# ishika28/Beyond-Binary-Fake-User-Detection-A-Credibility-Aware-Graph-based-Recommender-System

Measured on AMD Instinct MI355X. Metric: SpMM edges/sec + BPR steps/sec, |E|=50M d=64, 1/2/4/8 MI355X; %HBM roofline, higher is better.
Workload: dtype f32

## Files before the change

beyond-binary-fake-user-detection-a-credibility-aware-graph-based-recommender-system_amd/_lib.py:

```python
from __future__ import annotations

import ctypes
import os
import re
from pathlib import Path

import torch

PKG_DIR = Path(__file__).resolve().parent
LIB_PATH = Path(os.environ.get("BBGR_LIB", PKG_DIR / "lib" / "libbbgr.so"))
HEADER_PATH = PKG_DIR.parent / "include" / "bbgr.h"

BBGR_OK = 0
STATUS = {0: "BBGR_OK", -1: "BBGR_ERR_INVALID", -2: "BBGR_ERR_UNSUPPORTED",
          -3: "BBGR_ERR_HIP", -4: "BBGR_ERR_WORKSPACE"}

OP_GS, OP_METHOD_A, OP_J, OP_SYM = 0, 1, 2, 3
NEG_CAP = 65536

c_int32 = ctypes.c_int32
c_int64 = ctypes.c_int64
c_float = ctypes.c_float
c_double = ctypes.c_double
c_void_p = ctypes.c_void_p
# ... 211 lines not shown
        ("side", c_void_p), ("side_bytes", c_int64),
        ("n_records", c_int64), ("user_bytes", c_int64), ("item_bytes", c_int64),
        ("text_bytes", c_int64),
        ("out_rating", c_void_p), ("out_helpful", c_void_p), ("out_verified", c_void_p),
        ("out_timestamp", c_void_p), ("out_ts_valid", c_void_p),
        ("user_data", c_void_p), ("user_off", c_void_p),
        ("item_data", c_void_p), ("item_off", c_void_p),
        ("text_data", c_void_p), ("text_off", c_void_p),
    ]


class Pcg64State(ctypes.Structure):
    _fields_ = [
        ("state_hi", c_uint64), ("state_lo", c_uint64),
        ("inc_hi", c_uint64), ("inc_lo", c_uint64),
        ("has_uint32", c_int32), ("uinteger", ctypes.c_uint32),
    ]


class BatchArgs(ctypes.Structure):
    _fields_ = [
        ("batch", c_int64), ("users", c_void_p), ("pos", c_void_p), ("neg", c_void_p),
        ("n_users", c_int64), ("n_items", c_int64),
        ("user_indptr", c_void_p), ("user_indices", c_void_p),
        ("mask_u", c_void_p), ("mask_i", c_void_p),
        ("list", c_void_p), ("count", c_void_p),
        ("slot_map", c_void_p), ("slot_bits", c_void_p),
        ("g_u", c_void_p), ("g_i", c_void_p), ("g_side", c_void_p),
        ("ld_gu", c_int64), ("ld_gi", c_int64), ("ld_side", c_int64),
        ("d", c_int32),
    ]


class RowsMarkArgs(ctypes.Structure):
    _fields_ = [
        ("n_users_listed", c_int64), ("n_items_listed", c_int64),
        ("users", c_void_p), ("items", c_void_p),
        ("n_users", c_int64), ("n_items", c_int64),
        ("user_rank", c_void_p), ("item_rank", c_void_p),
        ("user_indptr", c_void_p), ("user_indices", c_void_p),
        ("mask_u", c_void_p), ("mask_i", c_void_p), ("frontier", c_void_p),
        ("mask_u_in", c_void_p), ("mask_i_in", c_void_p),
        ("user_list", c_void_p), ("user_count", c_void_p),
        ("frontier_list", c_void_p), ("frontier_count", c_void_p),
    ]


_P = c_void_p
_SIGNATURES = {
    "bbgr_abi_version": ([], c_int32),
    "bbgr_last_error": ([], ctypes.c_char_p),
    "bbgr_device_info": ([ctypes.c_int, _P, ctypes.c_char_p, ctypes.c_int], c_int32),
    "bbgr_sync": ([_P], c_int32),
    "bbgr_profile_marker": ([c_int32, _P], c_int32),
    "bbgr_csr_build": ([c_int64, _P, _P, c_int32, c_int32, _P, _P, _P, _P,
                        ctypes.POINTER(c_size_t), _P], c_int32),
    "bbgr_csr_plan_count": ([ctypes.POINTER(CsrStruct), ctypes.POINTER(c_int32),
                             ctypes.POINTER(c_int32), _P, ctypes.POINTER(c_size_t), _P],
                            c_int32),
    "bbgr_csr_plan_build": ([ctypes.POINTER(CsrStruct), _P, _P, _P,
                             ctypes.POINTER(c_size_t), _P], c_int32),
    "bbgr_operator_scales": ([c_int32, c_int32, c_int32, _P, _P, _P, _P, _P, _P, _P,
                              _P, _P, _P, _P, _P], c_int32),
    "bbgr_gather_scale": ([c_int64, _P, _P, _P, _P], c_int32),
    "bbgr_degree_count": ([c_int64, _P, c_int32, _P, _P], c_int32),
    "bbgr_degree_count_ws": ([c_int64, _P, c_int32, _P, _P, ctypes.POINTER(c_size_t), _P],
                             c_int32),
    "bbgr_degree_order": ([c_int32, _P, _P, _P, _P, ctypes.POINTER(c_size_t), _P], c_int32),
    "bbgr_relabel": ([c_int64, _P, _P, _P, _P], c_int32),
    "bbgr_spmm": ([ctypes.POINTER(CsrStruct), ctypes.POINTER(SpmmArgs), _P], c_int32),
    "bbgr_epilogue": ([c_int32, _P, c_int64, ctypes.POINTER(SpmmArgs), _P], c_int32),
    "bbgr_to_bf16": ([c_int64, c_int32, _P, c_int64, _P, c_int64, _P], c_int32),
    "bbgr_spmm_bf16": ([ctypes.POINTER(CsrStruct), ctypes.POINTER(SpmmArgs),
                        ctypes.POINTER(SpmmBf16Io), _P], c_int32),
    "bbgr_bpr": ([ctypes.POINTER(BprArgs), _P], c_int32),
    "bbgr_bpr_reduce": ([c_int64, _P, c_float, c_float, _P, _P], c_int32),
    "bbgr_adam": ([c_int64, _P, _P, _P, _P, c_float, c_double, c_double, c_float,
                   c_float, c_float, c_float, c_float, _P], c_int32),
    "bbgr_adam_dev": ([c_int64, _P, _P, _P, _P, c_float, c_double, c_double, c_float,
                       c_float, c_float, _P, _P, _P], c_int32),
    "bbgr_step_begin": ([_P, _P], c_int32),
    "bbgr_mark_rows": ([c_int64, _P, ctypes.c_uint8, _P, c_int64, _P], c_int32),
    "bbgr_comm_unique_id": ([_P], c_int32),
    "bbgr_comm_init": ([_P, c_int32, c_int32, _P], c_int32),
    "bbgr_comm_destroy": ([_P], c_int32),
    "bbgr_allreduce_items": ([_P, _P, c_int64, _P], c_int32),
    "bbgr_comm_allreduce": ([_P, _P, c_int64, c_int32, c_int32, _P], c_int32),
    "bbgr_comm_allgather": ([_P, _P, _P, c_int64, c_int32, _P], c_int32),
    "bbgr_ewa_normalize": ([ctypes.POINTER(CsrStruct), _P, _P, _P, _P, c_int64, c_int32, c_int32,
                            c_float, c_float, c_float, _P, _P, _P, _P,
                            ctypes.POINTER(c_size_t), _P], c_int32),
    "bbgr_scatter_add_rows": ([c_int64, _P, _P, c_int64, _P, c_int64, c_int32, c_int64, _P,
                               ctypes.POINTER(c_size_t), _P], c_int32),
    "bbgr_scatter_plan": ([c_int64, _P, c_int64, _P, ctypes.POINTER(c_size_t), _P], c_int32),
    "bbgr_scatter_apply": ([c_int64, c_int64, _P, _P, c_int64, _P, c_int64, _P, c_int64, c_int32,
                            _P], c_int32),
    "bbgr_mark_neighbors": ([c_int64, _P, _P, _P, ctypes.c_uint8, _P, _P], c_int32),
    "bbgr_mark_slots": ([c_int64, _P, _P, _P, _P, c_int32, _P], c_int32),
    "bbgr_batch_begin": ([ctypes.POINTER(BatchArgs), _P], c_int32),
    "bbgr_mask_pack": ([c_int64, _P, _P, _P], c_int32),
    "bbgr_batch_end": ([ctypes.POINTER(BatchArgs), _P], c_int32),
    "bbgr_rows_mark": ([ctypes.POINTER(RowsMarkArgs), _P], c_int32),
    "bbgr_mark_list": ([c_int64, _P, _P, _P, _P, c_int64, _P, _P, _P], c_int32),
    "bbgr_slots_from_perms": ([c_int64, _P, _P, _P, _P, _P], c_int32),
    "bbgr_transpose_slots": ([ctypes.POINTER(CsrStruct), ctypes.POINTER(CsrStruct), _P, _P],
                             c_int32),
    "bbgr_mark_neighbors_of_mask": ([c_int64, _P, _P, _P, _P, ctypes.c_uint8, _P, _P],
                                    c_int32),
    "bbgr_row_support": ([c_int64, c_int32, _P, c_int64, _P, _P, _P, _P, _P], c_int32),
    "bbgr_rows_zero": ([c_int64, _P, _P, c_int64, c_int32, _P], c_int32),
    "bbgr_rows_axpy": ([c_int64, _P, c_float, _P, c_int64, _P, c_int64, c_int32, _P],
                       c_int32),
    "bbgr_pop_cdf": ([c_int32, _P, c_double, _P, _P, ctypes.POINTER(c_size_t), _P],
                     c_int32),
# ... 165 lines not shown
```

beyond-binary-fake-user-detection-a-credibility-aware-graph-based-recommender-system_amd/csrc/common.h:

```cpp
#pragma once

#include <hip/hip_runtime.h>
#include <stdint.h>
#include <stdio.h>
#include <string>
#include <type_traits>

#include "bbgr.h"

namespace bbgr {

void set_error(const char *fmt, ...);

inline int hip_fail(hipError_t e, const char *what) {
  set_error("%s: %s", what, hipGetErrorString(e));
  return BBGR_ERR_HIP;
}

#define BBGR_HIP(call)                                                        \
  do {                                                                        \
    hipError_t e_ = (call);                                                   \
    if (e_ != hipSuccess) return ::bbgr::hip_fail(e_, #call);                 \
  } while (0)

// ... 94 lines not shown
    case 8: return f(std::integral_constant<int, 8>{});
    case 16: return f(std::integral_constant<int, 16>{});
    case 32: return f(std::integral_constant<int, 32>{});
    case 64: return f(std::integral_constant<int, 64>{});
    case 128: return f(std::integral_constant<int, 128>{});
    default: return f(std::integral_constant<int, 256>{});
  }
}

template <typename F> inline auto for_wide_width(int d, F &&f) {
  switch (d) {
    case 64: return f(std::integral_constant<int, 64>{});
    case 128: return f(std::integral_constant<int, 128>{});
    default: return f(std::integral_constant<int, 256>{});
  }
}

typedef float f4v __attribute__((ext_vector_type(4)));
__device__ __forceinline__ float4 ld_nt(const float4 *p) {
  const f4v v = __builtin_nontemporal_load(reinterpret_cast<const f4v *>(p));
  return make_float4(v.x, v.y, v.z, v.w);
}
__device__ __forceinline__ int ld_nt(const int *p) { return __builtin_nontemporal_load(p); }
__device__ __forceinline__ float ld_nt(const float *p) { return __builtin_nontemporal_load(p); }
__device__ __forceinline__ void st_nt(float4 *p, float4 v) {
  f4v w;
  w.x = v.x;
  w.y = v.y;
  w.z = v.z;
  w.w = v.w;
  __builtin_nontemporal_store(w, reinterpret_cast<f4v *>(p));
}

struct AdamConsts {
  float step;
  float w1;
  float b2;
  float w2;
  float eps;
  float wd;
  float bc2s;
};

__host__ __device__ inline AdamConsts adam_consts(float lr, double b1, double b2, float eps,
                                                  float wd, float bc1, float bc2s) {
  return AdamConsts{lr / bc1, (float)(1.0 - b1), (float)b2, (float)(1.0 - b2), eps, wd, bc2s};
}

__device__ __forceinline__ void adam_elem(float &p, float g, float &m, float &v,
                                          const AdamConsts &c) {
#pragma clang fp contract(off)
  if (c.wd != 0.f) g = fmaf(c.wd, p, g);
  m = fmaf(c.w1, g - m, m);
  v = fmaf(c.w2 * g, g, v * c.b2);
  const float denom = sqrtf(v) / c.bc2s + c.eps;
  p = fmaf(-c.step, m / denom, p);
}

__device__ __forceinline__ long clamp_step(const long *state) {
  const long t = state[0], n = state[3];
  return t < 1 ? 1 : (t > n ? n : t);
}

__host__ __device__ __forceinline__ int plan_chunks(long deg, int thr, int chunk) {
  return deg > thr ? (int)((deg + chunk - 1) / chunk) : 0;
}

}
```

beyond-binary-fake-user-detection-a-credibility-aware-graph-based-recommender-system_amd/csrc/train.hip:

```cpp
#include <hipcub/hipcub.hpp>

#include "common.h"

namespace bbgr {

struct BprParams {
  long batch, n_users, n_items;
  const long *users, *pos, *neg;
  const float *uf, *itf, *ue, *ie;
  long lduf, ldif, ldue, ldie;
  const float *pop;
  float reg, lambda_fair, inv_b;
  float *parts;
  const float *dloss;
  float *g_uf, *g_if, *g_ue, *g_ie;
  long ldguf, ldgif, ldgue, ldgie;
  float *contrib;
  long ldc;
  float *scores_out;
  const float *scores;
};

__device__ __forceinline__ float group16_sum(float v) {
  v += __shfl_xor(v, 1, 16);
// ... 214 lines not shown
#pragma unroll
    for (int u = 0; u < ADAM_TILE; ++u) {
      const long k = t0 + u * 256 + threadIdx.x;
      if (k < n4) {
        pp[u] = ld_nt(p + k);
        gg[u] = ld_nt(g + k);
        mm[u] = ld_nt(m + k);
        vv[u] = ld_nt(v + k);
      }
    }
#pragma unroll
    for (int u = 0; u < ADAM_TILE; ++u) {
      const long k = t0 + u * 256 + threadIdx.x;
      if (k < n4) {
        adam_elem(pp[u].x, gs * gg[u].x, mm[u].x, vv[u].x, c);
        adam_elem(pp[u].y, gs * gg[u].y, mm[u].y, vv[u].y, c);
        adam_elem(pp[u].z, gs * gg[u].z, mm[u].z, vv[u].z, c);
        adam_elem(pp[u].w, gs * gg[u].w, mm[u].w, vv[u].w, c);
        st_nt(p + k, pp[u]);
        st_nt(m + k, mm[u]);
        st_nt(v + k, vv[u]);
      }
    }
  }
}

__global__ void adam_tail_kernel(long n, long start, float *p, const float *g, float *m,
                                 float *v, AdamConsts c0, float gs, float lr, const float *bc,
                                 const long *state) {
  const long i = start + (long)blockIdx.x * blockDim.x + threadIdx.x;
  if (i >= n) return;
  const AdamConsts c = device_step_consts(c0, lr, bc, state);
  adam_elem(p[i], gs * g[i], m[i], v[i], c);
}

__global__ void step_begin_kernel(long *state) {
  if (threadIdx.x != 0 || blockIdx.x != 0) return;
  const long t = state[0], next = state[2];
  state[0] = t + 1;
  state[1] = next;
  state[2] = next + 1;
}

__global__ void rows_zero_kernel(long n, const long *idx, float *t, long ld,
                                 int d) {
  const long k = (long)blockIdx.x * (blockDim.x / 16) + (threadIdx.x >> 4);
  if (k >= n || idx[k] < 0) return;
  float *row = t + idx[k] * ld;
  for (int c = threadIdx.x & 15; c < d; c += 16) row[c] = 0.f;
}

__global__ void mark_rows_kernel(long n, const long *idx, unsigned char v,
                                 unsigned char *mask, long n_rows) {
  const long k = (long)blockIdx.x * blockDim.x + threadIdx.x;
  if (k >= n) return;
  const long r = idx[k];
  if (r >= 0 && r < n_rows) mask[r] = v;
}

__global__ void mark_neighbors_kernel(long n, const long *rows, const int *indptr,
                                      const int *indices, unsigned char v,
                                      unsigned char *mask) {
  const long k = (long)blockIdx.x * (blockDim.x / 16) + (threadIdx.x >> 4);
  if (k >= n || rows[k] < 0) return;
  const long r = rows[k];
  for (int e = indptr[r] + (threadIdx.x & 15); e < indptr[r + 1]; e += 16)
// ... 708 lines not shown
                       dim3(256), 0, st, (long)n, start, param, grad, exp_avg,
                       exp_avg_sq, c, grad_scale, lr, bc, state);
    BBGR_LAUNCHED("adam_tail_kernel");
  }
  return BBGR_OK;
}

extern "C" int bbgr_adam(int64_t n, float *param, const float *grad,
                         float *exp_avg, float *exp_avg_sq, float lr, double beta1,
                         double beta2, float eps, float weight_decay, float grad_scale,
                         float bias_correction1, float bias_correction2_sqrt,
                         bbgr_stream_t stream) {
  BBGR_REQUIRE(n >= 0, "bbgr_adam: negative n");
  if (n == 0) return BBGR_OK;
  BBGR_REQUIRE(param && grad && exp_avg && exp_avg_sq, "bbgr_adam: null tensor");
  return adam_launch(n, param, grad, exp_avg, exp_avg_sq, lr, beta1, beta2, eps, weight_decay,
                     grad_scale, bias_correction1, bias_correction2_sqrt, nullptr, nullptr,
                     as_stream(stream));
}

extern "C" int bbgr_adam_dev(int64_t n, float *param, const float *grad, float *exp_avg,
                             float *exp_avg_sq, float lr, double beta1, double beta2,
                             float eps, float weight_decay, float grad_scale,
                             const float *bc_table, const int64_t *state,
                             bbgr_stream_t stream) {
  BBGR_REQUIRE(n >= 0, "bbgr_adam_dev: negative n");
  if (n == 0) return BBGR_OK;
  BBGR_REQUIRE(param && grad && exp_avg && exp_avg_sq && bc_table && state,
               "bbgr_adam_dev: null tensor / table / state");
  return adam_launch(n, param, grad, exp_avg, exp_avg_sq, lr, beta1, beta2, eps, weight_decay,
                     grad_scale, 1.f, 1.f, bc_table, (const long *)state, as_stream(stream));
}

extern "C" int bbgr_step_begin(int64_t *state, bbgr_stream_t stream) {
  BBGR_REQUIRE(state, "bbgr_step_begin: null state");
  hipLaunchKernelGGL(step_begin_kernel, dim3(1), dim3(64), 0, as_stream(stream), (long *)state);
  BBGR_LAUNCHED("step_begin_kernel");
  return BBGR_OK;
}

extern "C" int bbgr_rows_zero(int64_t n, const int64_t *idx, float *table,
                              int64_t ld, int32_t d, bbgr_stream_t stream) {
  BBGR_REQUIRE(n >= 0 && d > 0 && ld >= d, "bbgr_rows_zero: bad sizes");
  if (n == 0) return BBGR_OK;
  BBGR_REQUIRE(idx && table, "bbgr_rows_zero: null arrays");
  hipLaunchKernelGGL(rows_zero_kernel, dim3((unsigned)((n + 15) / 16)), dim3(256), 0,
                     as_stream(stream), (long)n, (const long *)idx, table, (long)ld, d);
  BBGR_LAUNCHED("rows_zero_kernel");
  return BBGR_OK;
}

extern "C" int bbgr_mark_rows(int64_t n, const int64_t *idx, uint8_t value,
                              uint8_t *mask, int64_t n_rows, bbgr_stream_t stream) {
  BBGR_REQUIRE(n >= 0 && n_rows >= 0, "bbgr_mark_rows: negative n / n_rows");
  if (n == 0) return BBGR_OK;
  BBGR_REQUIRE(idx && mask, "bbgr_mark_rows: null arrays");
  hipLaunchKernelGGL(mark_rows_kernel, dim3((unsigned)((n + 255) / 256)), dim3(256), 0,
                     as_stream(stream), (long)n, (const long *)idx, value, mask, (long)n_rows);
  BBGR_LAUNCHED("mark_rows_kernel");
  return BBGR_OK;
}

extern "C" int bbgr_mark_neighbors(int64_t n, const int64_t *rows,
                                   const int32_t *indptr, const int32_t *indices,
                                   uint8_t value, uint8_t *mask, bbgr_stream_t stream) {
  BBGR_REQUIRE(n >= 0, "bbgr_mark_neighbors: negative n");
// ... 377 lines not shown
```

beyond-binary-fake-user-detection-a-credibility-aware-graph-based-recommender-system_amd/trainer.py:

```python
from __future__ import annotations

import ctypes
import os

import numpy as np
import torch

from . import _lib
from ._lib import OP_GS, OP_J, OP_METHOD_A, OP_SYM, call, ld, ptr, stream_handle
from .bpr import bpr_args
from .graph import BipartiteGraph, Csr
from .optim import AdamRows, DeviceStepState, adam_step
from .propagate import ORDER_GS, ORDER_J, ListLength, OperatorPair, backward, forward
from .sampler import PopMixSampler, nonempty_rows, shuffle
from .scatter import RowScatter

VARIANTS = {
    "v2_pop": (OP_GS, ORDER_GS, 0.7),
    "cu_message": (OP_GS, ORDER_GS, 0.0),
    "method_a": (OP_METHOD_A, ORDER_GS, 0.0),
    "cu_fair": (OP_J, ORDER_J, 0.0),
    "plain": (OP_SYM, ORDER_J, 0.0),
}

FRONTIER_MIN_EDGES = 500_000


def resolve_frontier(frontier, nnz: int) -> bool:
    if isinstance(frontier, str):
        if frontier != "auto":
            raise ValueError(f"frontier must be True, False or 'auto', got {frontier!r}")
        return nnz >= FRONTIER_MIN_EDGES
    return bool(frontier)


def default_tables(U: int, I: int, d: int, seed: int, user_seed: int | None = None,
                   user_fan: int | None = None):
    gi = torch.Generator(device="cpu").manual_seed(seed)
    gu = gi if user_seed is None else torch.Generator(device="cpu").manual_seed(user_seed)

    def draw(n, fan, g):
        return (torch.rand(n, d, generator=g) * 2 - 1) * (6.0 / (fan + d)) ** 0.5
    u0 = draw(U, U if user_fan is None else user_fan, gu)
    return u0, draw(I, I, gi)


FORWARD_DTYPES = {"fp32": torch.float32, "bf16": torch.bfloat16}


class FusedTrainer:
    forward_dtype, table_dtype = "fp32", torch.float32

    def __init__(self, graph: BipartiteGraph, variant: str = "v2_pop", cred=None,
                 emb_dim: int = 64, num_layers: int = 3, lr: float = 1e-3,
                 reg: float = 1e-4, batch_size: int = 4096, neg_mix_pop: float | None = None,
                 neg_pop_gamma: float = 0.75, neg_max_tries: int = 50,
                 lambda_fair: float = 0.0, seed: int = 42, u0=None, i0=None,
                 frontier="auto", fuse_adam: bool = True, forward_dtype: str = "fp32"):
        kind, mix = self._init_model(variant, graph.num_users, graph.num_items, emb_dim,
                                     num_layers, lr, reg, lambda_fair, seed, graph.device,
                                     forward_dtype, neg_mix_pop)
        self._init_operator(graph, kind, cred)
        if u0 is None:
            u0, i0 = default_tables(self.U, self.I, emb_dim, seed)
        self._init_tables(u0, i0, batch_size)
        self._init_batching(batch_size, graph.item_csr, mix, neg_pop_gamma, neg_max_tries, seed)
        self._init_step_state(frontier, graph.item_csr.nnz, fuse_adam)
        self._init_batch_buffers()

    def _init_model(self, variant: str, U: int, I: int, emb_dim: int, num_layers: int,
                    lr: float, reg: float, lambda_fair: float, seed: int, device,
                    forward_dtype: str, neg_mix_pop: float | None):
        if forward_dtype not in FORWARD_DTYPES:
            raise ValueError(f"forward_dtype must be 'fp32' or 'bf16', got {forward_dtype!r}")
        if forward_dtype == "bf16" and emb_dim < 64:
            raise ValueError(f"forward_dtype='bf16' needs emb_dim >= 64, got {emb_dim}")
        self.forward_dtype, self.table_dtype = forward_dtype, FORWARD_DTYPES[forward_dtype]
        _lib.require_gpu()
        if variant not in VARIANTS:
            raise ValueError(f"unknown variant {variant!r}; one of {sorted(VARIANTS)}")
        kind, self.order, mix_default = VARIANTS[variant]
        self.variant, self.device = variant, device
        self.U, self.I, self.d, self.K = U, I, emb_dim, num_layers
        self.lr, self.reg, self.lambda_fair, self.seed = lr, reg, lambda_fair, seed
        return kind, mix_default if neg_mix_pop is None else neg_mix_pop

    def _init_operator(self, graph: BipartiteGraph, kind: int, cred, scales=None) -> None:
        self.graph = graph
        cred_t = None
        if cred is not None and kind != OP_SYM:
            cred_t = torch.as_tensor(np.asarray(cred, np.float32)).to(self.device).contiguous()
            cred_t = _internal_rows(graph.user_order, cred_t)
        self.scales = graph.scales(kind, cred_t) if scales is None else scales(cred_t)
        self.pair = OperatorPair.factored(graph, self.scales)

    def _init_tables(self, u0, i0, B: int, item_moment_rows: int | None = None) -> None:
        graph, d = self.graph, self.d
        f32 = dict(dtype=torch.float32, device=self.device)
        self.user_w = torch.as_tensor(u0, dtype=torch.float32).to(self.device).contiguous()
        self.item_w = torch.as_tensor(i0, dtype=torch.float32).to(self.device).contiguous()
        if self.user_w.shape != (self.U, d) or self.item_w.shape != (self.I, d):
# ... 65 lines not shown
                and os.environ.get("BBGR_MASK_BITS", "1") != "0"):
            self.mask_i_bits = torch.zeros(self.I // 32 + 1, dtype=torch.int32, device=dev)
        self.batch_fused = (self.frontier and order == ORDER_GS
                            and os.environ.get("BBGR_BATCH_FUSED", "1") != "0")
        if self.frontier and order == ORDER_GS:
            self.item_list = torch.empty(max(self.I, 1), dtype=torch.int64, device=dev)
            self.item_count = torch.zeros(1, dtype=torch.int64, device=dev)
            self.item_len = ListLength(self.item_count, wait=num_layers >= 2)

    def enable_device_state(self, max_steps: int = 1 << 20) -> None:
        if self.dev_state is None:
            self.dev_state = DeviceStepState(self.device, self.step_count, self.sampler.counter,
                                             max_steps)

    def next_users(self) -> torch.Tensor:
        n = self.train_users.numel()
        if self.perm is None or self.cursor >= n:
            self.epoch += 1
            self.perm = shuffle(self.train_users, self.seed, self.epoch)
            self.cursor = 0
        users = self.perm[self.cursor: self.cursor + self.B]
        self.cursor += self.B
        return users

    def step(self, users: torch.Tensor | None = None) -> torch.Tensor:
        listed = users is None
        if users is None:
            users = self.next_users()
        else:
            users = users.to(device=self.device, dtype=torch.int64)
            if self.graph.user_order is not None:
                users = self.graph.user_order.to_internal(users)
            users = users.contiguous()
        return self._step(users, listed)

    def _step(self, users: torch.Tensor, listed: bool) -> torch.Tensor:
        if self.dev_state is not None:
            self.dev_state.begin()
        self._last_users = users
        B = users.numel()
        self.pos, self.neg = self.posneg[:B], self.posneg[B:2 * B]
        pos, neg = self.sampler.sample(users, self.pos, self.neg,
                                       state=None if self.dev_state is None
                                       else self.dev_state.state)
        st = stream_handle()
        masks = self._set_masks(users, pos, neg, 1) if self.frontier else None
        forward(self.pair, self.user_w, self.item_w, self.K, self.order, out_u=self.uf,
                out_i=self.itf, ws=self.ws,
                final_rows=None if masks is None else
                (masks[0], masks[1], users if listed else None, self._flist(masks)),
                tag=self._tag(masks), table_dtype=self.table_dtype)
        self._bpr(users, pos, neg, B)
        self.scatter(self.g_uf, users, self.contrib[:B], unique=listed)
        self.scatter(self.g_if, self.posneg[: 2 * B], self.contrib[B: 3 * B])
        call("bbgr_bpr_reduce", B, ptr(self.parts), float(self.reg), float(self.lambda_fair),
             ptr(self.loss), st)
        alpha = 2.0 * self.reg / B
        if self.fuse_adam and self.order == ORDER_J:
            self._backward_fused_j(users, self.posneg[: 2 * B], masks, alpha)
        elif self.fuse_adam:
            self._backward_fused(users, self.posneg[: 2 * B], masks, alpha)
        else:
            backward(self.pair, self.g_uf, self.g_if, self.K, self.order, out_u=self.g_u0,
                     out_i=self.g_i0, ws=self.ws, grad_support=masks,
                     src_bits=self._bits(masks), frontier_list=self._flist(masks),
                     tagged=self._tagged(masks), item_mask_bits=self._mask_bits(masks))
            self._unfused_tail(users, (pos, neg), alpha)
        if self._fused_pending:
            self._fused_pending = False
            a = self._batch_args(users, g=True)
            call("bbgr_batch_end", ctypes.byref(a), st)
            self.item_len.invalidate()
            return self.loss
        call("bbgr_rows_zero", B, ptr(users), ptr(self.g_uf), ld(self.g_uf), self.d, st)
        call("bbgr_rows_zero", 2 * B, ptr(self.posneg), ptr(self.g_if), ld(self.g_if), self.d,
             st)
        if masks is not None:
            self._set_masks(users, pos, neg, 0)
# ... 23 lines not shown
        a.user_indptr, a.user_indices = ptr(uc.indptr), ptr(uc.indices)
        a.mask_u, a.mask_i = ptr(self.mask_u), ptr(self.mask_i)
        a.list, a.count = ptr(self.item_list), ptr(self.item_count)
        if bits is not None:
            a.slot_map, a.slot_bits = ptr(self.slot_map), ptr(bits)
        if g:
            a.g_u, a.ld_gu = ptr(self.g_uf), ld(self.g_uf)
            a.g_i, a.ld_gi = ptr(self.g_if), ld(self.g_if)
            if side is not None:
                a.g_side, a.ld_side = ptr(side), ld(side)
        a.d = self.d
        return a

    def _bpr(self, users, pos, neg, B: int) -> None:
        a = bpr_args(users, pos, neg, self.uf, self.itf, self.user_w, self.item_w, self.reg,
                     self.pop, self.lambda_fair, parts=self.parts[: 3 * B],
                     contrib=self.contrib)
        call("bbgr_bpr", ctypes.byref(a), stream_handle())

    def _backward_fused(self, users, item_rows, masks, alpha: float, reduce=None,
                        item_adam: bool = True) -> None:
        st = stream_handle()
        B = users.numel()
        gl = 1.0 / (self.K + 1)
        a_gl = alpha / gl
        self.step_count += 1
        adam_u = AdamRows(self.user_w, self.m_u, self.v_u, self.step_count, self.lr,
                          dev=self.dev_state)

        def before_last():
            call("bbgr_rows_axpy", B, ptr(users), a_gl, ptr(self.user_w), ld(self.user_w),
                 ptr(self.g_uf), ld(self.g_uf), self.d, st)

        side = item_adam and reduce is None and self.K >= 2
        adam_i = None
        if side:
            ga = self._item_grad_side()
            call("bbgr_rows_copy", item_rows.numel(), ptr(item_rows), ptr(self.g_if),
                 ld(self.g_if), ptr(ga), ld(ga), self.d, st)
            call("bbgr_rows_axpy", item_rows.numel(), ptr(item_rows), a_gl, ptr(self.item_w),
                 ld(self.item_w), ptr(ga), ld(ga), self.d, st)
            adam_i = AdamRows(self.item_w, self.m_i, self.v_i, self.step_count, self.lr,
                              dev=self.dev_state, grad=ga, grad_scale=gl)
        backward(self.pair, self.g_uf, self.g_if, self.K, self.order, out_u=self.g_u0,
                 ws=self.ws, grad_support=masks, grad_i0_dense=False, adam_u=adam_u,
                 src_bits=self._bits(masks), frontier_list=self._flist(masks),
                 before_last=before_last, reduce=reduce, adam_i=adam_i,
                 tagged=self._tagged(masks), item_mask_bits=self._mask_bits(masks))
        if side:
            if not self._fused_pending:
                call("bbgr_rows_zero", item_rows.numel(), ptr(item_rows), ptr(ga), ld(ga),
                     self.d, st)
        elif item_adam:
            self._item_adam(item_rows, self.g_if, a_gl, gl)

    def _item_grad_side(self) -> torch.Tensor:
        if self._g_item_side is None:
            self._g_item_side = torch.zeros_like(self.g_if)
        return self._g_item_side

    def _item_adam(self, item_rows, g, a_gl: float, gl: float) -> None:
        st = stream_handle()
        call("bbgr_rows_axpy", item_rows.numel(), ptr(item_rows), a_gl, ptr(self.item_w),
             ld(self.item_w), ptr(g), ld(g), self.d, st)
        adam_step(self.item_w, g, self.m_i, self.v_i, self.step_count, self.lr,
                  grad_scale=gl, dev=self.dev_state)

    def _backward_fused_j(self, users, item_rows, masks, alpha: float) -> None:
        st = stream_handle()
        B = users.numel()
        a_gl = alpha / (1.0 / (self.K + 1))
        self.step_count += 1
        adam_u = AdamRows(self.user_w, self.m_u, self.v_u, self.step_count, self.lr,
                          dev=self.dev_state)
        adam_i = AdamRows(self.item_w, self.m_i, self.v_i, self.step_count, self.lr,
                          dev=self.dev_state)

        def before_last():
            call("bbgr_rows_axpy", B, ptr(users), a_gl, ptr(self.user_w), ld(self.user_w),
                 ptr(self.g_uf), ld(self.g_uf), self.d, st)
            call("bbgr_rows_axpy", item_rows.numel(), ptr(item_rows), a_gl, ptr(self.item_w),
                 ld(self.item_w), ptr(self.g_if), ld(self.g_if), self.d, st)
# ... 100 lines not shown
    def recommend(self, users, k: int, exclude_train: bool = True, item_mask=None,
                  return_scores: bool = False, precision: str = "fp32", **kw):
        from .recommend import recommend
        uf, itf = self.forward()
        return recommend(uf, itf, users, k, exclude=self._train_rows() if exclude_train else None,
                         item_mask=item_mask, return_scores=return_scores, precision=precision,
                         **kw)

    def batch(self):
        B = self._last_users.numel()
        users, pos, neg = self._last_users, self.posneg[:B], self.posneg[B:2 * B]
        go, gi = self.graph.user_order, self.graph.item_order
        if go is not None:
            users = go.to_input(users)
        if gi is not None:
            pos, neg = gi.to_input(pos), gi.to_input(neg)
        return users, pos, neg

    def state_dict(self) -> dict:
        return {"user_emb.weight": _input_rows(self.graph.user_order, self.user_w),
                "item_emb.weight": _input_rows(self.graph.item_order, self.item_w)}


class GraphedStep:

    def __init__(self, trainer: FusedTrainer):
        self.tr = trainer
        trainer.enable_device_state()
        self.first_loss = None
        if trainer.step_count == 0:
            self.first_loss = trainer.step()
        self.users = torch.zeros(trainer.B, dtype=torch.int64, device=trainer.device)
        host = (trainer.step_count, trainer.sampler.counter)
        self._captured = (trainer.frontier, trainer.fuse_adam, trainer.B, trainer.forward_dtype)
        trainer.pair.prepare_graph(trainer.d)
        torch.cuda.synchronize()
        self.graph = torch.cuda.CUDAGraph()
        with torch.cuda.graph(self.graph):
            trainer._step(self.users, True)
        trainer.step_count, trainer.sampler.counter = host
        torch.cuda.synchronize()

    def step(self) -> torch.Tensor:
        tr = self.tr
        if (tr.frontier, tr.fuse_adam, tr.B, tr.forward_dtype) != self._captured:
            raise RuntimeError("GraphedStep: the trainer's frontier / fuse_adam / batch size / "
                               "forward_dtype changed since capture; build a new GraphedStep")
        users = tr.next_users()
        if users.numel() != tr.B:
            return tr._step(users, True)
        self.users.copy_(users)
        self.graph.replay()
        tr.step_count += 1
        tr.sampler.counter += 1
        tr._last_users = self.users
        tr.pos, tr.neg = tr.posneg[: tr.B], tr.posneg[tr.B: 2 * tr.B]
        return tr.loss


def _internal_rows(order, t: torch.Tensor) -> torch.Tensor:
    return t if order is None else order.rows_to_internal(t)


def _input_rows(order, t: torch.Tensor) -> torch.Tensor:
    return t if order is None else order.rows_to_input(t)
```

include/bbgr.h:

```cpp
#ifndef BBGR_H
#define BBGR_H

#include <stddef.h>
#include <stdint.h>

#ifdef __cplusplus
extern "C" {
#endif

#define BBGR_ABI_VERSION 12

typedef enum {
  BBGR_OK = 0,
  BBGR_ERR_INVALID = -1,
  BBGR_ERR_UNSUPPORTED = -2,
  BBGR_ERR_HIP = -3,
  BBGR_ERR_WORKSPACE = -4
} bbgr_status;

typedef void *bbgr_stream_t;

int bbgr_abi_version(void);
const char *bbgr_last_error(void);
int bbgr_device_info(int device, int *cu_count, char *arch_name, int arch_name_len);
// ... 153 lines not shown
  const float *itf; int64_t ldif;
  const float *ue; int64_t ldue;
  const float *ie; int64_t ldie;
  const float *pop;
  float reg;
  float lambda_fair;
  float *parts;
  const float *dloss;
  float *g_uf; int64_t ldguf;
  float *g_if; int64_t ldgif;
  float *g_ue; int64_t ldgue;
  float *g_ie; int64_t ldgie;
  float *contrib; int64_t ldcontrib;
  float *scores_out;
  const float *scores;
} bbgr_bpr_args;

int bbgr_bpr(const bbgr_bpr_args *args, bbgr_stream_t stream);

int bbgr_bpr_reduce(int64_t batch, const float *parts, float reg,
                    float lambda_fair, float *loss, bbgr_stream_t stream);

int bbgr_adam(int64_t n, float *param, const float *grad, float *exp_avg,
              float *exp_avg_sq, float lr, double beta1, double beta2, float eps,
              float weight_decay, float grad_scale, float bias_correction1,
              float bias_correction2_sqrt, bbgr_stream_t stream);

int bbgr_step_begin(int64_t *state, bbgr_stream_t stream);
int bbgr_adam_dev(int64_t n, float *param, const float *grad, float *exp_avg,
                  float *exp_avg_sq, float lr, double beta1, double beta2, float eps,
                  float weight_decay, float grad_scale, const float *bc_table,
                  const int64_t *state, bbgr_stream_t stream);

int bbgr_rows_zero(int64_t n, const int64_t *idx, float *table, int64_t ld,
                   int32_t d, bbgr_stream_t stream);
int bbgr_rows_axpy(int64_t n, const int64_t *idx, float alpha, const float *src,
                   int64_t ldsrc, float *dst, int64_t lddst, int32_t d,
                   bbgr_stream_t stream);

int bbgr_rows_copy(int64_t n, const int64_t *idx, const float *src, int64_t ldsrc,
                   float *dst, int64_t lddst, int32_t d, bbgr_stream_t stream);

int bbgr_rows_gather(int64_t n, const int64_t *idx, const float *src, int64_t ldsrc,
                     float *dst, int64_t lddst, int32_t d, bbgr_stream_t stream);

int bbgr_rows_add_unique(int64_t n, const int64_t *idx, const float *src, int64_t ldsrc,
                         float *dst, int64_t lddst, int32_t d, int64_t n_dst,
                         bbgr_stream_t stream);

int bbgr_first_slot(int64_t n, const int64_t *ids, int64_t n_rows, int32_t *first,
                    int64_t *slot, bbgr_stream_t stream);

int bbgr_ego_slots(int64_t B, const int64_t *users, const int64_t *pos, const int64_t *neg,
                   int64_t n_users, int64_t n_items, int32_t *first_u, int32_t *first_i,
                   int64_t *iu, int64_t *ii, int64_t *cu, int64_t *sp, int64_t *sn,
                   bbgr_stream_t stream);

int bbgr_ego_rows(int64_t B, int32_t d, const int64_t *cu, const int64_t *sp, const int64_t *sn,
                  const int64_t *iu, const int64_t *ii, const float *ue, int64_t ldue,
                  const float *ie, int64_t ldie, const float *dloss, float reg, int32_t *counts,
                  float *g_u, int64_t ldgu, float *g_i, int64_t ldgi, float scale,
                  int32_t *counts_u_out, bbgr_stream_t stream);

int bbgr_rows_add_slots(int64_t n, const int64_t *slot, const int32_t *counts,
                        const int64_t *rows, const float *src, int64_t ldsrc, float *dst,
                        int64_t lddst, int32_t d, int64_t n_dst, bbgr_stream_t stream);
// ... 486 lines not shown
```

Before: 27.32 billion.

## Add lazy per-row item Adam with catch-up replay and periodic flush

```diff
diff --git a/beyond-binary-fake-user-detection-a-credibility-aware-graph-based-recommender-system_amd/_lib.py b/beyond-binary-fake-user-detection-a-credibility-aware-graph-based-recommender-system_amd/_lib.py
--- a/beyond-binary-fake-user-detection-a-credibility-aware-graph-based-recommender-system_amd/_lib.py
+++ b/beyond-binary-fake-user-detection-a-credibility-aware-graph-based-recommender-system_amd/_lib.py
@@ -267,6 +267,22 @@
     ]
 
 
+class LazyAdamArgs(ctypes.Structure):
+    _fields_ = [
+        ("n_rows", c_int64),
+        ("param", c_void_p), ("exp_avg", c_void_p), ("exp_avg_sq", c_void_p),
+        ("ld", c_int64), ("d", c_int32),
+        ("last_step", c_void_p), ("occurrences", c_void_p),
+        ("n", c_int64), ("rows", c_void_p),
+        ("grad", c_void_p), ("ld_grad", c_int64),
+        ("grad_scale", c_float), ("ego_scale", c_float),
+        ("lr", c_float), ("eps", c_float), ("weight_decay", c_float),
+        ("beta1", c_double), ("beta2", c_double),
+        ("bc_table", c_void_p), ("bc_steps", c_int64),
+        ("step", c_int64), ("state", c_void_p),
+    ]
+
+
 class RowsMarkArgs(ctypes.Structure):
     _fields_ = [
         ("n_users_listed", c_int64), ("n_items_listed", c_int64),
@@ -315,6 +331,9 @@
     "bbgr_adam_dev": ([c_int64, _P, _P, _P, _P, c_float, c_double, c_double, c_float,
                        c_float, c_float, _P, _P, _P], c_int32),
     "bbgr_step_begin": ([_P, _P], c_int32),
+    "bbgr_adam_rows_catchup": ([ctypes.POINTER(LazyAdamArgs), _P], c_int32),
+    "bbgr_adam_rows_step": ([ctypes.POINTER(LazyAdamArgs), _P], c_int32),
+    "bbgr_adam_flush": ([ctypes.POINTER(LazyAdamArgs), _P], c_int32),
     "bbgr_mark_rows": ([c_int64, _P, ctypes.c_uint8, _P, c_int64, _P], c_int32),
     "bbgr_comm_unique_id": ([_P], c_int32),
     "bbgr_comm_init": ([_P, c_int32, c_int32, _P], c_int32),
diff --git a/beyond-binary-fake-user-detection-a-credibility-aware-graph-based-recommender-system_amd/csrc/adam_elem.h b/beyond-binary-fake-user-detection-a-credibility-aware-graph-based-recommender-system_amd/csrc/adam_elem.h
--- /dev/null
+++ b/beyond-binary-fake-user-detection-a-credibility-aware-graph-based-recommender-system_amd/csrc/adam_elem.h
@@ -0,0 +1,71 @@
+#pragma once
+
+#include <math.h>
+
+#if defined(__HIPCC__)
+#define BBGR_HD __host__ __device__ __forceinline__
+#else
+#define BBGR_HD inline
+#endif
+
+namespace bbgr {
+
+struct AdamConsts {
+  float step;
+  float w1;
+  float b2;
+  float w2;
+  float eps;
+  float wd;
+  float bc2s;
+};
+
+BBGR_HD AdamConsts adam_consts(float lr, double b1, double b2, float eps, float wd, float bc1,
+                               float bc2s) {
+  return AdamConsts{lr / bc1, (float)(1.0 - b1), (float)b2, (float)(1.0 - b2), eps, wd, bc2s};
+}
+
+BBGR_HD void adam_elem(float &p, float g, float &m, float &v, const AdamConsts &c) {
+#if defined(__clang__)
+#pragma clang fp contract(off)
+#endif
+  if (c.wd != 0.f) g = fmaf(c.wd, p, g);
+  m = fmaf(c.w1, g - m, m);
+  v = fmaf(c.w2 * g, g, v * c.b2);
+  const float denom = sqrtf(v) / c.bc2s + c.eps;
+  p = fmaf(-c.step, m / denom, p);
+}
+
+BBGR_HD AdamConsts table_step_consts(AdamConsts c, float lr, const float *bc, long n_bc, long s) {
+  const long k = s < 1 ? 1 : (s > n_bc ? n_bc : s);
+  c.step = lr / bc[2 * (k - 1)];
+  c.bc2s = bc[2 * (k - 1) + 1];
+  return c;
+}
+
+template <int N>
+BBGR_HD void adam_replay(float (&p)[N], float (&m)[N], float (&v)[N], float g0,
+                         const AdamConsts &base, float lr, const float *bc, long n_bc, long s0,
+                         long s1) {
+  for (long s = s0 + 1; s <= s1; ++s) {
+    const AdamConsts c = table_step_consts(base, lr, bc, n_bc, s);
+#if defined(__clang__)
+#pragma unroll
+#endif
+    for (int j = 0; j < N; ++j) adam_elem(p[j], g0, m[j], v[j], c);
+  }
+}
+
+constexpr int LAZY_GROUP = 16;
+constexpr int LAZY_BLOCK = 256;
+constexpr int LAZY_COLS = 4;
+BBGR_HD int lazy_col_of(int lane, int pass, int slot) {
+  return lane + LAZY_GROUP * (pass * LAZY_COLS + slot);
+}
+BBGR_HD long lazy_blocks(long n) { return (n + LAZY_GROUP - 1) / LAZY_GROUP; }
+BBGR_HD long lazy_group_of(long block, int thread) {
+  return block * (LAZY_BLOCK / LAZY_GROUP) + (thread / LAZY_GROUP);
+}
+BBGR_HD int lazy_lane_of(int thread) { return thread % LAZY_GROUP; }
+
+}
diff --git a/beyond-binary-fake-user-detection-a-credibility-aware-graph-based-recommender-system_amd/csrc/common.h b/beyond-binary-fake-user-detection-a-credibility-aware-graph-based-recommender-system_amd/csrc/common.h
--- a/beyond-binary-fake-user-detection-a-credibility-aware-graph-based-recommender-system_amd/csrc/common.h
+++ b/beyond-binary-fake-user-detection-a-credibility-aware-graph-based-recommender-system_amd/csrc/common.h
@@ -150,30 +150,9 @@
   __builtin_nontemporal_store(w, reinterpret_cast<f4v *>(p));
 }
 
-struct AdamConsts {
-  float step;
-  float w1;
-  float b2;
-  float w2;
-  float eps;
-  float wd;
-  float bc2s;
-};
-
-__host__ __device__ inline AdamConsts adam_consts(float lr, double b1, double b2, float eps,
-                                                  float wd, float bc1, float bc2s) {
-  return AdamConsts{lr / bc1, (float)(1.0 - b1), (float)b2, (float)(1.0 - b2), eps, wd, bc2s};
 }
-
-__device__ __forceinline__ void adam_elem(float &p, float g, float &m, float &v,
-                                          const AdamConsts &c) {
-#pragma clang fp contract(off)
-  if (c.wd != 0.f) g = fmaf(c.wd, p, g);
-  m = fmaf(c.w1, g - m, m);
-  v = fmaf(c.w2 * g, g, v * c.b2);
-  const float denom = sqrtf(v) / c.bc2s + c.eps;
-  p = fmaf(-c.step, m / denom, p);
-}
+#include "adam_elem.h"
+namespace bbgr {
 
 __device__ __forceinline__ long clamp_step(const long *state) {
   const long t = state[0], n = state[3];
diff --git a/beyond-binary-fake-user-detection-a-credibility-aware-graph-based-recommender-system_amd/csrc/train.hip b/beyond-binary-fake-user-detection-a-credibility-aware-graph-based-recommender-system_amd/csrc/train.hip
--- a/beyond-binary-fake-user-detection-a-credibility-aware-graph-based-recommender-system_amd/csrc/train.hip
+++ b/beyond-binary-fake-user-detection-a-credibility-aware-graph-based-recommender-system_amd/csrc/train.hip
@@ -270,6 +270,124 @@
   if (i >= n) return;
   const AdamConsts c = device_step_consts(c0, lr, bc, state);
   adam_elem(p[i], gs * g[i], m[i], v[i], c);
+}
+
+struct LazyAdamParams {
+  long n_rows, n, ld, ld_g, n_bc, step;
+  float *p, *m, *v;
+  int *last_step, *occ;
+  const long *rows, *state;
+  const float *bc, *g;
+  AdamConsts base;
+  float lr, gs, ego;
+  int d;
+};
+
+__device__ __forceinline__ long lazy_step(const LazyAdamParams &P) {
+  return P.state ? P.state[0] : P.step;
+}
+
+struct LazyCols {
+  float p[LAZY_COLS], m[LAZY_COLS], v[LAZY_COLS];
+};
+
+__device__ __forceinline__ void lazy_load(const LazyAdamParams &P, long r, int lane, int q,
+                                          LazyCols &x) {
+#pragma unroll
+  for (int j = 0; j < LAZY_COLS; ++j) {
+    const int c = lazy_col_of(lane, q, j);
+    const bool in = c < P.d;
+    const long k = r * P.ld + c;
+    x.p[j] = in ? P.p[k] : 0.f;
+    x.m[j] = in ? P.m[k] : 0.f;
+    x.v[j] = in ? P.v[k] : 0.f;
+  }
+}
+
+__device__ __forceinline__ void lazy_store(const LazyAdamParams &P, long r, int lane, int q,
+                                           const LazyCols &x) {
+#pragma unroll
+  for (int j = 0; j < LAZY_COLS; ++j) {
+    const int c = lazy_col_of(lane, q, j);
+    if (c >= P.d) continue;
+    const long k = r * P.ld + c;
+    P.p[k] = x.p[j];
+    P.m[k] = x.m[j];
+    P.v[k] = x.v[j];
+  }
+}
+
+__device__ __forceinline__ void lazy_replay_row(const LazyAdamParams &P, long r, int lane,
+                                                long s0, long s1) {
+  const float g0 = P.gs * 0.0f;
+  for (int q = 0; lazy_col_of(lane, q, 0) < P.d; ++q) {
+    LazyCols x;
+    lazy_load(P, r, lane, q, x);
+    adam_replay<LAZY_COLS>(x.p, x.m, x.v, g0, P.base, P.lr, P.bc, P.n_bc, s0, s1);
+    lazy_store(P, r, lane, q, x);
+  }
+}
+
+__global__ __launch_bounds__(LAZY_BLOCK) void adam_rows_catchup_kernel(LazyAdamParams P) {
+  const long k = lazy_group_of(blockIdx.x, threadIdx.x);
+  const int lane = lazy_lane_of(threadIdx.x);
+  const long r = k < P.n ? P.rows[k] : -1;
+  const bool ok = r >= 0 && r < P.n_rows;
+  int seen = 1, ls = 0;
+  if (ok && lane == 0) {
+    ls = P.last_step[r];
+    seen = atomicAdd(P.occ + r, 1);
+  }
+  seen = __shfl(seen, 0, LAZY_GROUP);
+  ls = __shfl(ls, 0, LAZY_GROUP);
+  const long t1 = lazy_step(P) - 1;
+  if (!ok || seen != 0 || ls >= t1) return;
+  lazy_replay_row(P, r, lane, ls, t1);
+  if (lane == 0) P.last_step[r] = (int)t1;
+}
+
+__global__ __launch_bounds__(LAZY_BLOCK) void adam_rows_step_kernel(LazyAdamParams P) {
+  const long k = lazy_group_of(blockIdx.x, threadIdx.x);
+  const int lane = lazy_lane_of(threadIdx.x);
+  const long r = k < P.n ? P.rows[k] : -1;
+  const bool ok = r >= 0 && r < P.n_rows;
+  int n = 0;
+  if (ok && lane == 0) n = atomicExch(P.occ + r, 0);
+  n = __shfl(n, 0, LAZY_GROUP);
+  if (n <= 0) return;
+  const long t = lazy_step(P);
+  const AdamConsts c = table_step_consts(P.base, P.lr, P.bc, P.n_bc, t);
+  for (int q = 0; lazy_col_of(lane, q, 0) < P.d; ++q) {
+    LazyCols x;
+    lazy_load(P, r, lane, q, x);
+    float acc[LAZY_COLS], ego[LAZY_COLS];
+#pragma unroll
+    for (int j = 0; j < LAZY_COLS; ++j) {
+      const int col = lazy_col_of(lane, q, j);
+      acc[j] = col < P.d ? P.g[r * P.ld_g + col] : 0.f;
+      ego[j] = __fmul_rn(P.ego, x.p[j]);
+    }
+    for (int i = 0; i < n; ++i) {
+#pragma unroll
+      for (int j = 0; j < LAZY_COLS; ++j) acc[j] = __fadd_rn(acc[j], ego[j]);
+    }
+#pragma unroll
+    for (int j = 0; j < LAZY_COLS; ++j)
+      adam_elem(x.p[j], __fmul_rn(P.gs, acc[j]), x.m[j], x.v[j], c);
+    lazy_store(P, r, lane, q, x);
+  }
+  if (lane == 0) P.last_step[r] = (int)t;
+}
+
+__global__ __launch_bounds__(LAZY_BLOCK) void adam_flush_kernel(LazyAdamParams P) {
+  const long r = lazy_group_of(blockIdx.x, threadIdx.x);
+  const int lane = lazy_lane_of(threadIdx.x);
+  if (r >= P.n_rows) return;
+  const long t = lazy_step(P);
+  const int ls = P.last_step[r];
+  if (ls >= t) return;
+  lazy_replay_row(P, r, lane, ls, t);
+  if (lane == 0) P.last_step[r] = (int)t;
 }
 
 __global__ void step_begin_kernel(long *state) {
@@ -1044,6 +1162,71 @@
                      grad_scale, 1.f, 1.f, bc_table, (const long *)state, as_stream(stream));
 }
 
+static int lazy_adam_launch(const char *who, const bbgr_lazy_adam_args *a, int which,
+                            bbgr_stream_t stream) {
+  BBGR_REQUIRE_IN(who, a != nullptr, "null args");
+  BBGR_REQUIRE_IN(who, a->n_rows >= 0 && a->d > 0 && a->ld >= a->d, "bad table sizes");
+  BBGR_REQUIRE_IN(who, a->n_rows <= 0x7fffffffL * LAZY_GROUP, "too many rows");
+  BBGR_REQUIRE_IN(who, a->bc_steps >= 1 && a->bc_table, "needs the bias-correction table");
+  BBGR_REQUIRE_IN(who, a->state || (a->step >= (which == 2 ? 0 : 1) && a->step <= 0x7fffffffL),
+                  "step out of range (and no device state)");
+  const long n = which == 2 ? a->n_rows : a->n;
+  BBGR_REQUIRE_IN(who, n >= 0 && n <= 0x7fffffffL * LAZY_GROUP, "bad row count");
+  if (n == 0 || a->n_rows == 0) return BBGR_OK;
+  BBGR_REQUIRE_IN(who, a->param && a->exp_avg && a->exp_avg_sq && a->last_step,
+                  "null table / stamps");
+  LazyAdamParams P{};
+  P.n_rows = a->n_rows;
+  P.n = n;
+  P.ld = a->ld;
+  P.d = a->d;
+  P.p = a->param;
+  P.m = a->exp_avg;
+  P.v = a->exp_avg_sq;
+  P.last_step = a->last_step;
+  P.bc = a->bc_table;
+  P.n_bc = a->bc_steps;
+  P.step = a->step;
+  P.state = (const long *)a->state;
+  P.lr = a->lr;
+  P.gs = a->grad_scale;
+  P.base = adam_consts(a->lr, a->beta1, a->beta2, a->eps, a->weight_decay, 1.f, 1.f);
+  const dim3 grid((unsigned)lazy_blocks(n)), block(LAZY_BLOCK);
+  hipStream_t st = as_stream(stream);
+  if (which == 2) {
+    hipLaunchKernelGGL(adam_flush_kernel, grid, block, 0, st, P);
+    BBGR_LAUNCHED("adam_flush_kernel");
+    return BBGR_OK;
+  }
+  BBGR_REQUIRE_IN(who, a->rows && a->occurrences, "null row list / occurrence counts");
+  P.rows = (const long *)a->rows;
+  P.occ = a->occurrences;
+  if (which == 0) {
+    hipLaunchKernelGGL(adam_rows_catchup_kernel, grid, block, 0, st, P);
+    BBGR_LAUNCHED("adam_rows_catchup_kernel");
+    return BBGR_OK;
+  }
+  BBGR_REQUIRE_IN(who, a->grad && a->ld_grad >= a->d, "null gradient table / bad ld_grad");
+  P.g = a->grad;
+  P.ld_g = a->ld_grad;
+  P.ego = a->ego_scale;
+  hipLaunchKernelGGL(adam_rows_step_kernel, grid, block, 0, st, P);
+  BBGR_LAUNCHED("adam_rows_step_kernel");
+  return BBGR_OK;
+}
+
+extern "C" int bbgr_adam_rows_catchup(const bbgr_lazy_adam_args *a, bbgr_stream_t stream) {
+  return lazy_adam_launch("bbgr_adam_rows_catchup", a, 0, stream);
+}
+
+extern "C" int bbgr_adam_rows_step(const bbgr_lazy_adam_args *a, bbgr_stream_t stream) {
+  return lazy_adam_launch("bbgr_adam_rows_step", a, 1, stream);
+}
+
+extern "C" int bbgr_adam_flush(const bbgr_lazy_adam_args *a, bbgr_stream_t stream) {
+  return lazy_adam_launch("bbgr_adam_flush", a, 2, stream);
+}
+
 extern "C" int bbgr_step_begin(int64_t *state, bbgr_stream_t stream) {
   BBGR_REQUIRE(state, "bbgr_step_begin: null state");
   hipLaunchKernelGGL(step_begin_kernel, dim3(1), dim3(64), 0, as_stream(stream), (long *)state);
diff --git a/beyond-binary-fake-user-detection-a-credibility-aware-graph-based-recommender-system_amd/trainer.py b/beyond-binary-fake-user-detection-a-credibility-aware-graph-based-recommender-system_amd/trainer.py
--- a/beyond-binary-fake-user-detection-a-credibility-aware-graph-based-recommender-system_amd/trainer.py
+++ b/beyond-binary-fake-user-detection-a-credibility-aware-graph-based-recommender-system_amd/trainer.py
@@ -1,6 +1,7 @@
 from __future__ import annotations
 
 import ctypes
+import math
 import os
 
 import numpy as np
@@ -10,7 +11,7 @@
 from ._lib import OP_GS, OP_J, OP_METHOD_A, OP_SYM, call, ld, ptr, stream_handle
 from .bpr import bpr_args
 from .graph import BipartiteGraph, Csr
-from .optim import AdamRows, DeviceStepState, adam_step
+from .optim import AdamRows, DeviceStepState, adam_step, exact_table_steps
 from .propagate import ORDER_GS, ORDER_J, ListLength, OperatorPair, backward, forward
 from .sampler import PopMixSampler, nonempty_rows, shuffle
 from .scatter import RowScatter
@@ -47,9 +48,12 @@
 
 FORWARD_DTYPES = {"fp32": torch.float32, "bf16": torch.bfloat16}
 
+LAZY_FLUSH_EVERY = 64
+
 
 class FusedTrainer:
     forward_dtype, table_dtype = "fp32", torch.float32
+    _lazy = _in_step = False
 
     def __init__(self, graph: BipartiteGraph, variant: str = "v2_pop", cred=None,
                  emb_dim: int = 64, num_layers: int = 3, lr: float = 1e-3,
@@ -67,6 +71,64 @@
         self._init_batching(batch_size, graph.item_csr, mix, neg_pop_gamma, neg_max_tries, seed)
         self._init_step_state(frontier, graph.item_csr.nnz, fuse_adam)
         self._init_batch_buffers()
+        if type(self) is FusedTrainer:
+            self._init_lazy_item_adam()
+
+    def _item_state(self, name: str, new: torch.Tensor | None = None) -> torch.Tensor:
+        if self._lazy and not self._in_step:
+            self._lazy_flush()
+        if new is not None:
+            self.__dict__[name] = new
+        return self.__dict__[name]
+
+    item_w = property(lambda self: self._item_state("_item_w"),
+                      lambda self, t: self._item_state("_item_w", t))
+    m_i = property(lambda self: self._item_state("_m_i"),
+                   lambda self, t: self._item_state("_m_i", t))
+    v_i = property(lambda self: self._item_state("_v_i"),
+                   lambda self, t: self._item_state("_v_i", t))
+
+    def _init_lazy_item_adam(self) -> None:
+        if not (self.fuse_adam and self.order == ORDER_GS and self.K >= 2
+                and os.environ.get("BBGR_LAZY_ITEM_ADAM", "1") != "0"):
+            return
+        self.lazy_flush_every = max(1, int(os.environ.get("BBGR_LAZY_FLUSH_EVERY",
+                                                          LAZY_FLUSH_EVERY)))
+        i32 = dict(dtype=torch.int32, device=self.device)
+        self._lazy_stamp = torch.full((self.I,), self.step_count, **i32)
+        self._lazy_occ = torch.zeros(self.I, **i32)
+        self._lazy_flushed_at = self.step_count
+        b1, b2 = 0.9, 0.999
+        bc = np.array([(1.0 - b1 ** t, math.sqrt(1.0 - b2 ** t))
+                       for t in range(1, exact_table_steps(b1, b2) + 1)], dtype=np.float64)
+        self._lazy_bc = torch.from_numpy(bc.astype(np.float32)).to(self.device)
+        self._lazy = True
+
+    def _lazy_args(self, step: int):
+        w = self.__dict__["_item_w"]
+        a = _lib.LazyAdamArgs()
+        a.n_rows, a.ld, a.d = self.I, ld(w), self.d
+        a.param, a.exp_avg = ptr(w), ptr(self.__dict__["_m_i"])
+        a.exp_avg_sq = ptr(self.__dict__["_v_i"])
+        a.last_step, a.occurrences = ptr(self._lazy_stamp), ptr(self._lazy_occ)
+        a.lr, a.eps, a.weight_decay, a.beta1, a.beta2 = self.lr, 1e-8, 0.0, 0.9, 0.999
+        a.grad_scale = 1.0 / (self.K + 1)
+        bc = self._lazy_bc if self.dev_state is None else self.dev_state.bc_table
+        a.bc_table, a.bc_steps, a.step = ptr(bc), bc.shape[0], step
+        if self.dev_state is not None:
+            a.state = ptr(self.dev_state.state)
+        return a
+
+    def _lazy_flush(self) -> None:
+        if self._lazy_flushed_at == self.step_count:
+            return
+        a = self._lazy_args(self.step_count)
+        call("bbgr_adam_flush", ctypes.byref(a), stream_handle())
+        self._lazy_flushed_at = self.step_count
+
+    def _lazy_flush_if_due(self) -> None:
+        if self._lazy and self.step_count - self._lazy_flushed_at >= self.lazy_flush_every:
+            self._lazy_flush()
 
     def _init_model(self, variant: str, U: int, I: int, emb_dim: int, num_layers: int,
                     lr: float, reg: float, lambda_fair: float, seed: int, device,
@@ -198,9 +260,17 @@
             if self.graph.user_order is not None:
                 users = self.graph.user_order.to_internal(users)
             users = users.contiguous()
+        self._lazy_flush_if_due()
         return self._step(users, listed)
 
     def _step(self, users: torch.Tensor, listed: bool) -> torch.Tensor:
+        self._in_step = True
+        try:
+            return self._step_launches(users, listed)
+        finally:
+            self._in_step = False
+
+    def _step_launches(self, users: torch.Tensor, listed: bool) -> torch.Tensor:
         if self.dev_state is not None:
             self.dev_state.begin()
         self._last_users = users
@@ -210,6 +280,10 @@
                                        state=None if self.dev_state is None
                                        else self.dev_state.state)
         st = stream_handle()
+        if self._lazy:
+            a = self._lazy_args(self.step_count + 1)
+            a.n, a.rows = 2 * B, ptr(self.posneg)
+            call("bbgr_adam_rows_catchup", ctypes.byref(a), st)
         masks = self._set_masks(users, pos, neg, 1) if self.frontier else None
         forward(self.pair, self.user_w, self.item_w, self.K, self.order, out_u=self.uf,
                 out_i=self.itf, ws=self.ws,
@@ -299,7 +373,8 @@
             call("bbgr_rows_axpy", B, ptr(users), a_gl, ptr(self.user_w), ld(self.user_w),
                  ptr(self.g_uf), ld(self.g_uf), self.d, st)
 
-        side = item_adam and reduce is None and self.K >= 2
+        lazy = self._lazy and item_adam and reduce is None
+        side = item_adam and reduce is None and self.K >= 2 and not lazy
         adam_i = None
         if side:
             ga = self._item_grad_side()
@@ -314,7 +389,12 @@
                  src_bits=self._bits(masks), frontier_list=self._flist(masks),
                  before_last=before_last, reduce=reduce, adam_i=adam_i,
                  tagged=self._tagged(masks), item_mask_bits=self._mask_bits(masks))
-        if side:
+        if lazy:
+            a = self._lazy_args(self.step_count)
+            a.n, a.rows = item_rows.numel(), ptr(item_rows)
+            a.grad, a.ld_grad, a.ego_scale = ptr(self.g_if), ld(self.g_if), a_gl
+            call("bbgr_adam_rows_step", ctypes.byref(a), st)
+        elif side:
             if not self._fused_pending:
                 call("bbgr_rows_zero", item_rows.numel(), ptr(item_rows), ptr(ga), ld(ga),
                      self.d, st)
@@ -481,7 +561,8 @@
             self.first_loss = trainer.step()
         self.users = torch.zeros(trainer.B, dtype=torch.int64, device=trainer.device)
         host = (trainer.step_count, trainer.sampler.counter)
-        self._captured = (trainer.frontier, trainer.fuse_adam, trainer.B, trainer.forward_dtype)
+        self._captured = (trainer.frontier, trainer.fuse_adam, trainer.B, trainer.forward_dtype,
+                          trainer._lazy)
         trainer.pair.prepare_graph(trainer.d)
         torch.cuda.synchronize()
         self.graph = torch.cuda.CUDAGraph()
@@ -492,9 +573,10 @@
 
     def step(self) -> torch.Tensor:
         tr = self.tr
-        if (tr.frontier, tr.fuse_adam, tr.B, tr.forward_dtype) != self._captured:
+        if (tr.frontier, tr.fuse_adam, tr.B, tr.forward_dtype, tr._lazy) != self._captured:
             raise RuntimeError("GraphedStep: the trainer's frontier / fuse_adam / batch size / "
                                "forward_dtype changed since capture; build a new GraphedStep")
+        tr._lazy_flush_if_due()
         users = tr.next_users()
         if users.numel() != tr.B:
             return tr._step(users, True)
diff --git a/include/bbgr.h b/include/bbgr.h
--- a/include/bbgr.h
+++ b/include/bbgr.h
@@ -209,6 +209,29 @@
                   float weight_decay, float grad_scale, const float *bc_table,
                   const int64_t *state, bbgr_stream_t stream);
 
+typedef struct {
+  int64_t n_rows;
+  float *param, *exp_avg, *exp_avg_sq;
+  int64_t ld;
+  int32_t d;
+  int32_t *last_step;
+  int32_t *occurrences;
+  int64_t n;
+  const int64_t *rows;
+  const float *grad;
+  int64_t ld_grad;
+  float grad_scale, ego_scale;
+  float lr, eps, weight_decay;
+  double beta1, beta2;
+  const float *bc_table;
+  int64_t bc_steps;
+  int64_t step;
+  const int64_t *state;
+} bbgr_lazy_adam_args;
+int bbgr_adam_rows_catchup(const bbgr_lazy_adam_args *args, bbgr_stream_t stream);
+int bbgr_adam_rows_step(const bbgr_lazy_adam_args *args, bbgr_stream_t stream);
+int bbgr_adam_flush(const bbgr_lazy_adam_args *args, bbgr_stream_t stream);
+
 int bbgr_rows_zero(int64_t n, const int64_t *idx, float *table, int64_t ld,
                    int32_t d, bbgr_stream_t stream);
 int bbgr_rows_axpy(int64_t n, const int64_t *idx, float alpha, const float *src,
```

Measured after the change: 27.55 billion (median of 6 runs). No clear change (+0.8%).
